# mgp25/OpenLTE

Hardware: AMD Instinct MI355X
Metric: DL subframes/sec @20MHz 100RB 64QAM, full chain FFT->CE->demap->rate-unmatch->turbo(REF)->CRC (SURVEY 8d W4) (higher is better)
Workload: dtype i8 IQ in, f32 FFT/CE/equaliser, i8 soft bits, i16 path metrics (differences exact modulo 2^16); 1 GPU; W4 full DL chain: 20 MHz/100 RB/64QAM, 9 allocations per subframe (8x12 PRB TBS 3240 + 1x4 PRB TBS 1064), 65536 subframes per GPU, int8 IQ in HBM; subframes_per_gpu=65536, N_ant=1, CFI=2, channel_estimate_form=compact, decoder=REF (reference-faithful, bit-exact), unique_subframes=96, streams_per_gpu=1

## Files before the change

### openlte_amd/csrc/turbo.hip

```cpp
#include <algorithm>
#include <cstring>
#include <initializer_list>
#include <type_traits>
#include <vector>

#include "plan_core.hpp"
#include "turbo_swar.h"

using namespace turbo_geom;

namespace {

constexpr uint32_t RX_NULL_AS_INT = 10000;


__device__ __forceinline__ int sbyte(uint32_t w, int k) { return (int)__builtin_amdgcn_sbfe(w, 8 * k, 8); }

typedef __attribute__((address_space(3))) const uint8_t  lds_u8_t;
typedef __attribute__((address_space(3))) const int8_t   lds_i8_t;
typedef __attribute__((address_space(3))) const uint16_t lds_u16_t;
__device__ __forceinline__ uint32_t lds_u8(uint32_t addr) { return *(lds_u8_t *)(uintptr_t)addr; }
__device__ __forceinline__ int      lds_i8(uint32_t addr) { return *(lds_i8_t *)(uintptr_t)addr; }
__device__ __forceinline__ uint32_t lds_u16(uint32_t addr) { return *(lds_u16_t *)(uintptr_t)addr; }

// ... 663 lines not shown
            mtab1[t] = (int8_t)(int)(127.0f * (w / W1));
            mtab2[t] = (int8_t)(int)(127.0f * (w / W2));
        }
        __syncthreads();
    }
    if (nv >= 0) {
        *reinterpret_cast<uint4 *>(out.arr[4] + unit_off(tile_off, lane, u)) = closed(w1max) ? closed16(w1, w1max) : lookup16(0, w1);
        *reinterpret_cast<uint4 *>(out.arr[5] + unit_off(tile_off, lane, u)) = closed(w2max) ? closed16(w2, w2max) : lookup16(MTAB_N, w2);
    }
}


struct SisoPass {
    const uint8_t *in_a;
    const uint8_t *in_b;
    const uint8_t *mag;
    uint8_t       *out;
    uint32_t      *dec;
};
struct SisoArgs { SisoPass p[2]; };

typedef unsigned short v2u __attribute__((ext_vector_type(2)));
__device__ __forceinline__ uint32_t sign_bits(v2s n) { return __builtin_bit_cast(uint32_t, __builtin_bit_cast(v2u, n) >> 15); }

template <int S> __device__ __forceinline__ void acs_step2(v2s (&pm)[8], v2s x2, v2s y2, uint32_t &acc)
{
    const v2s mx = as_v2s(neg_mask(x2 ^ y2)), nmx = ~mx;
    const v2s uP = (x2 + y2) & nmx;
    const v2s uQ = (x2 - y2) & mx;
    const uint32_t m0p = neg_mask(x2) & 0xFFF8FFF8u;
    const v2s P2 = as_v2s(__builtin_amdgcn_bitop3_b32(as_u32(mx), m0p, 0xFFFCFFFCu, 0x06));
    const v2s Q2 = as_v2s(__builtin_amdgcn_bitop3_b32(as_u32(mx), m0p, 0xFFFCFFFCu, 0x60));
// ... 10 lines not shown
    nw[1] = sel(n1 - Q2, pm[3] + uQ, pm[2] - uQ);
    nw[5] = sel(n1 + Q2, pm[3] - uQ, pm[2] + uQ);
    nw[2] = sel(n2 + Q2, pm[5] - uQ, pm[4] + uQ);
    nw[6] = sel(n2 - Q2, pm[5] + uQ, pm[4] - uQ);
    nw[3] = sel(n3 + P2, pm[7] - uP, pm[6] + uP);
    nw[7] = sel(n3 - P2, pm[7] + uP, pm[6] - uP);
#pragma unroll
    for (int s = 0; s < 8; s++) pm[s] = nw[s];
}

template <int R> __device__ __forceinline__ v2s byte_pair2(uint32_t w0, uint32_t w1)
{
    return as_v2s(__builtin_amdgcn_perm(w1, w0, (uint32_t)(4 + R) << 24 | 0x0C0000u | (uint32_t)R << 8 | 0x0Cu)) >> 7;
}

__device__ __forceinline__ uint32_t traceback_entry(uint32_t byte, uint32_t cur)
{
    uint32_t mask = 0;
    for (int k = 0; k < 2; k++) {
        const uint32_t nib = k ? byte >> 4 : byte & 15u;
        const uint32_t j = cur & 3u, bit = (nib >> (3 - j)) & 1u, st = 2 * j + bit;
        const bool     pos = (cur < st) || (cur == st && cur == 0);
        if (!pos) mask |= k ? 0x00FFu : 0xFF00u;
        cur = st;
    }
    return cur | mask << 8;
}

#ifndef SISO_WPE
#define SISO_WPE 4
#endif
template <bool MULTI>
__global__ __launch_bounds__(256) __attribute__((amdgpu_waves_per_eu(SISO_WPE, 8))) void k_turbo_siso(SisoArgs args, uint32_t K_arg, uint32_t n_tiles_arg, uint32_t mode, MultiArgs ma,
                                                                                                         const uint32_t *__restrict__ order)
{
    __shared__ uint32_t tb_lut[2048];
    for (uint32_t i = threadIdx.x; i < 2048; i += blockDim.x) tb_lut[i] = traceback_entry(i >> 3, i & 7u);
    __syncthreads();
    const uint32_t lane = threadIdx.x & 63u;
    uint32_t       K = K_arg, n_tiles = n_tiles_arg, wv = blockIdx.x * 4 + (threadIdx.x >> 6), n_wv = mode ? n_tiles : (n_tiles + 1) / 2;
    size_t         seg_off = 0;
    if constexpr (MULTI) {
        if (order) wv = __builtin_amdgcn_readfirstlane(order[wv]);
        if (wv >= n_tiles_arg) return;
        const_seg_t &sg = multi_seg(ma, wv);
        K = sg.K; n_tiles = sg.n_tiles; seg_off = sg.arr_off;
        wv -= mode ? sg.wv23 : sg.wv1;
        n_wv = mode ? n_tiles : (n_tiles + 1) / 2;
    }
    const uint32_t Kp = kpad64(K), nblk = Kp >> 6;
    if (wv >= n_wv) return;
    const uint8_t *pa[2], *pb[2], *pmag[2];
    uint8_t       *pout[2];
    uint32_t      *dec[2];
#pragma unroll
    for (int h = 0; h < 2; h++) {
        const SisoPass &ps   = args.p[mode ? h : 0];
        const uint32_t  tile = mode ? wv : min(2 * wv + h, n_tiles - 1);
        const size_t    off  = seg_off + (size_t)tile * Kp * 64 + lane * 64;
        pa[h] = ps.in_a + off; pb[h] = ps.in_b + off; pmag[h] = ps.mag + off; pout[h] = ps.out + off;
        dec[h] = ps.dec + (seg_off >> 3) + ((size_t)tile * nblk * 64 + lane) * 8;
    }

    v2s pm[8];
#pragma unroll
    for (int s = 0; s < 8; s++) pm[s] = (v2s)(0);

    uint4 A[2][4], B[2][4];
#pragma unroll
    for (int h = 0; h < 2; h++)
#pragma unroll
        for (int q = 0; q < 4; q++) {
            A[h][q] = reinterpret_cast<const uint4 *>(pa[h])[q];
            B[h][q] = reinterpret_cast<const uint4 *>(pb[h])[q];
        }
    for (uint32_t blk = 0; blk < nblk; blk++) {
        const uint32_t nxt = (blk + 1 < nblk) ? blk + 1 : blk;
        uint32_t       dw[2][8];
#pragma unroll
        for (int q = 0; q < 4; q++) {
#pragma unroll
            for (int g2 = 0; g2 < 2; g2++) {
                const int g = 2 * q + g2;
                uint32_t  acc_lo = 0, acc_hi = 0;
                if (blk * 64 + g * 8 < K) {
                    const uint32_t a0l = g2 ? A[0][q].z : A[0][q].x, a0h = g2 ? A[0][q].w : A[0][q].y;
                    const uint32_t a1l = g2 ? A[1][q].z : A[1][q].x, a1h = g2 ? A[1][q].w : A[1][q].y;
                    const uint32_t b0l = g2 ? B[0][q].z : B[0][q].x, b0h = g2 ? B[0][q].w : B[0][q].y;
                    const uint32_t b1l = g2 ? B[1][q].z : B[1][q].x, b1h = g2 ? B[1][q].w : B[1][q].y;
                    acs_step2<0>(pm, byte_pair2<0>(a0l, a1l), byte_pair2<0>(b0l, b1l), acc_lo);
                    acs_step2<1>(pm, byte_pair2<1>(a0l, a1l), byte_pair2<1>(b0l, b1l), acc_lo);
                    acs_step2<2>(pm, byte_pair2<2>(a0l, a1l), byte_pair2<2>(b0l, b1l), acc_lo);
                    acs_step2<3>(pm, byte_pair2<3>(a0l, a1l), byte_pair2<3>(b0l, b1l), acc_lo);
                    acs_step2<0>(pm, byte_pair2<0>(a0h, a1h), byte_pair2<0>(b0h, b1h), acc_hi);
                    acs_step2<1>(pm, byte_pair2<1>(a0h, a1h), byte_pair2<1>(b0h, b1h), acc_hi);
                    acs_step2<2>(pm, byte_pair2<2>(a0h, a1h), byte_pair2<2>(b0h, b1h), acc_hi);
                    acs_step2<3>(pm, byte_pair2<3>(a0h, a1h), byte_pair2<3>(b0h, b1h), acc_hi);
                }
                dw[0][g] = __builtin_amdgcn_perm(acc_lo, acc_hi, 0x05040100u);
                dw[1][g] = __builtin_amdgcn_perm(acc_lo, acc_hi, 0x07060302u);
            }
            if (q >= 2) {
#pragma unroll
                for (int qq = (q == 2 ? 0 : 3); qq <= (q == 2 ? 2 : 3); qq++)
#pragma unroll
                    for (int h = 0; h < 2; h++) {
                        A[h][qq] = reinterpret_cast<const uint4 *>(pa[h] + (size_t)nxt * 4096)[qq];
                        B[h][qq] = reinterpret_cast<const uint4 *>(pb[h] + (size_t)nxt * 4096)[qq];
                    }
            }
        }
#pragma unroll
        for (int h = 0; h < 2; h++) {
            uint4 *dp = reinterpret_cast<uint4 *>(dec[h] + (size_t)blk * 64 * 8);
            dp[0] = make_uint4(dw[h][0], dw[h][1], dw[h][2], dw[h][3]);
            dp[1] = make_uint4(dw[h][4], dw[h][5], dw[h][6], dw[h][7]);
        }
    }

    int cur[2] = {0, 0};
    {
        int best[2] = {0, 0};
#pragma unroll
        for (int s = 1; s < 8; s++) {
            const uint32_t d  = as_u32(pm[s] - pm[0]);
            const int      dh[2] = {(int)__builtin_amdgcn_sbfe(d, 0, 16), (int)d >> 16};
#pragma unroll
            for (int h = 0; h < 2; h++)
                if (dh[h] < best[h]) { best[h] = dh[h]; cur[h] = s; }
        }
    }

    uint4 M[2][4], Mn[2][4], D[2][2], Dn[2][2];
#pragma unroll
    for (int h = 0; h < 2; h++) {
        const uint4 *dp = reinterpret_cast<const uint4 *>(dec[h] + (size_t)(nblk - 1) * 64 * 8);
        D[h][0] = dp[0];
        D[h][1] = dp[1];
#pragma unroll
        for (int q = 0; q < 4; q++) M[h][q] = reinterpret_cast<const uint4 *>(pmag[h] + (size_t)(nblk - 1) * 4096)[q];
    }
    for (int blk = (int)nblk - 1; blk >= 0; blk--) {
        const int prv = blk > 0 ? blk - 1 : 0;
#pragma unroll
        for (int h = 0; h < 2; h++) {
            const uint4 *dpn = reinterpret_cast<const uint4 *>(dec[h] + (size_t)prv * 64 * 8);
            Dn[h][0] = dpn[0];
            Dn[h][1] = dpn[1];
#pragma unroll
            for (int q = 0; q < 4; q++) Mn[h][q] = reinterpret_cast<const uint4 *>(pmag[h] + (size_t)prv * 4096)[q];
        }
#pragma unroll
        for (int q = 3; q >= 0; q--) {
            uint32_t ow[2][4];
#pragma unroll
            for (int g2 = 1; g2 >= 0; g2--) {
                const int g = 2 * q + g2;
                uint32_t  o_hi[2] = {0, 0}, o_lo[2] = {0, 0};
                if ((uint32_t)blk * 64 + g * 8 < K) {
                    uint32_t word[2], mlo[2], mhi[2], msk[2][4];
#pragma unroll
                    for (int h = 0; h < 2; h++) {
                        const uint4 dq = D[h][g >> 2];
                        word[h] = (g & 3) == 0 ? dq.x : (g & 3) == 1 ? dq.y : (g & 3) == 2 ? dq.z : dq.w;
                        mlo[h]  = g2 ? M[h][q].z : M[h][q].x;
                        mhi[h]  = g2 ? M[h][q].w : M[h][q].y;
                    }
#pragma unroll
                    for (int b = 0; b < 4; b++) {
#pragma unroll
                        for (int h = 0; h < 2; h++) {
                            const uint32_t e = tb_lut[((word[h] >> (8 * b)) & 0xFFu) << 3 | (uint32_t)cur[h]];
                            cur[h]    = (int)(e & 7u);
                            msk[h][b] = e >> 8;
                        }
                    }
#pragma unroll
                    for (int h = 0; h < 2; h++) {
                        o_hi[h] = turbo_swar::joined_from(mhi[h], msk[h][0] << 16 | msk[h][1]);
                        o_lo[h] = turbo_swar::joined_from(mlo[h], msk[h][2] << 16 | msk[h][3]);
                    }
                }
#pragma unroll
                for (int h = 0; h < 2; h++) { ow[h][2 * g2] = o_lo[h]; ow[h][2 * g2 + 1] = o_hi[h]; }
            }
#pragma unroll
            for (int h = 0; h < 2; h++)
                reinterpret_cast<uint4 *>(pout[h] + (size_t)blk * 4096)[q] = make_uint4(ow[h][0], ow[h][1], ow[h][2], ow[h][3]);
        }
#pragma unroll
        for (int h = 0; h < 2; h++) {
            D[h][0] = Dn[h][0];
            D[h][1] = Dn[h][1];
#pragma unroll
            for (int q = 0; q < 4; q++) M[h][q] = Mn[h][q];
        }
    }
}

struct SmallPar { uint32_t cw, uw; };

__device__ __forceinline__ uint2 map_compose(uint2 F, uint2 G)
{
    return make_uint2(__builtin_amdgcn_perm(F.y, F.x, G.x), __builtin_amdgcn_perm(F.y, F.x, G.y));
}
__device__ __forceinline__ uint32_t map_at(uint2 F, uint32_t s) { return ((s & 4u ? F.y : F.x) >> (8 * (s & 3u))) & 7u; }
template <int N> __device__ __forceinline__ uint2 map_row_shl(uint2 v, uint2 keep)
{
    return make_uint2((uint32_t)__builtin_amdgcn_update_dpp((int)keep.x, (int)v.x, 0x100 + N, 0xF, 0xF, false),
                      (uint32_t)__builtin_amdgcn_update_dpp((int)keep.y, (int)v.y, 0x100 + N, 0xF, 0xF, false));
// ... 98 lines not shown
    {
        const uint32_t q0 = (uint32_t)__builtin_amdgcn_mov_dpp((int)XY, 0x00, 0xF, 0xF, false), q1 = (uint32_t)__builtin_amdgcn_mov_dpp((int)XY, 0x55, 0xF, 0xF, false);
        const uint32_t q2 = (uint32_t)__builtin_amdgcn_mov_dpp((int)XY, 0xAA, 0xF, 0xF, false), q3 = (uint32_t)__builtin_amdgcn_mov_dpp((int)XY, 0xFF, 0xF, 0xF, false);
        const short pm[8] = {(short)q0, (short)q1, (short)q2, (short)q3, (short)(q0 >> 16), (short)(q1 >> 16), (short)(q2 >> 16), (short)(q3 >> 16)};
        int best = 0;
#pragma unroll
        for (int st = 1; st < 8; st++) {
            const int d = (short)(pm[st] - pm[0]);
            if (d < best) { best = d; cur = st; }
        }
    }

    const uint2 MAP_ID = make_uint2(0x03020100u, 0x07060504u);
    for (uint32_t g = 0; g < n_g; g++) {
        uint32_t       end = (uint32_t)__builtin_amdgcn_readlane((int)cur, (int)(g * 4));
        const uint8_t *mag = pass_of(g).mag + off_of(g);
        uint8_t       *out = pass_of(g).out + off_of(g);
        uint8_t m_nxt = mag[(size_t)(n_chunk - 1) * 4096 + lane];
        for (int ch = (int)n_chunk - 1; ch >= 0; ch--) {
            const uint32_t t = (uint32_t)ch * 64 + lane;
            const uint8_t  m = m_nxt;
            if (ch > 0) m_nxt = mag[(size_t)(ch - 1) * 4096 + lane];
            const uint4    w = *reinterpret_cast<const uint4 *>(&decw[(g * n_w32 + (t >> 5)) * 4]);
            const uint32_t sh = 31u - (t & 31u);
            uint2          G = MAP_ID;
            if (t < K) {
                const uint32_t f = 0x06040200u + (((w.x >> sh) & 1u) | ((w.y >> sh) & 1u) << 8 | ((w.z >> sh) & 1u) << 16 | ((w.w >> sh) & 1u) << 24);
                G = make_uint2(f, f);
            }
            G = map_compose(G, map_row_shl<1>(G, MAP_ID));
            G = map_compose(G, map_row_shl<2>(G, MAP_ID));
            G = map_compose(G, map_row_shl<4>(G, MAP_ID));
            G = map_compose(G, map_row_shl<8>(G, MAP_ID));
            const uint32_t row = lane >> 4;
#pragma unroll
            for (int r = 1; r < 4; r++) {
                const uint2 R = make_uint2((uint32_t)__builtin_amdgcn_readlane((int)G.x, 16 * r), (uint32_t)__builtin_amdgcn_readlane((int)G.y, 16 * r));
                if (row < (uint32_t)r) G = map_compose(G, R);
            }
            const uint2    Gn  = make_uint2((uint32_t)__shfl_down((int)G.x, 1u), (uint32_t)__shfl_down((int)G.y, 1u));
            const uint32_t nxt = lane == 63 ? end : map_at(Gn, end);
            const uint32_t st  = map_at(G, end);
            if (t < K) {
                const bool    pos = (nxt < st) || (nxt == st && nxt == 0);
                out[(size_t)ch * 4096 + lane] = (pos || m == 0) ? m : (uint8_t)(m | 0x80u);
            }
            end = (uint32_t)__builtin_amdgcn_readlane((int)st, 0);
        }
    }
}

namespace sw = turbo_swar;
struct UnitWords { uint32_t w[5]; };
__device__ __forceinline__ UnitWords load_unit_words(const uint8_t *arr, size_t tile_off, uint32_t lane, uint32_t u)
{
    const uint4 c    = *reinterpret_cast<const uint4 *>(arr + unit_off(tile_off, lane, u));
    uint32_t    prev = 0x7F7F7F7Fu;
    if (u > 0) prev = *reinterpret_cast<const uint32_t *>(arr + unit_off(tile_off, lane, u - 1) + 12);
    return UnitWords{{prev, c.x, c.y, c.z, c.w}};
}
struct PermArgs { const uint8_t *A1; const uint8_t *X2; uint8_t *out[2];  };

#ifndef PERM_NB
#define PERM_NB 4
#endif
static_assert(PERM_NB == PERM_BLOCKS, "a size's perm grid is a multiple of 128 workgroups (the merged decode's map granularity) only for four blocks per workgroup");
template <int NSLOT, bool MULTI = false>
__global__ __launch_bounds__(384) void k_turbo_perm(PermArgs a, uint32_t K_arg, uint32_t n_cb_arg, const uint16_t *__restrict__ pi_arg, MultiArgs ma)
{
    static_assert(NSLOT == 1, "one unit per thread");
    uint32_t K = K_arg, n_cb = n_cb_arg, bidx = blockIdx.x, grid = gridDim.x;
    size_t   seg_off = 0;
    const uint16_t *__restrict__ pi = pi_arg;
    if constexpr (MULTI) {
        const_seg_t &sg = multi_seg(ma, blockIdx.x >> 7);
        K = sg.K; n_cb = sg.n_cb; pi = (const uint16_t *)sg.pi; bidx = blockIdx.x - sg.wg_perm; grid = sg.perm_grid;
// ... 15 lines not shown
#pragma unroll 1
    for (uint32_t it = 0; it < PERM_NB; it++) {
        const uint32_t cb = xcd_cb(bidx + it * grid, n_cb), tile = cb >> 6, lane = cb & 63;
        const size_t   tile_off = seg_off + (size_t)tile * Kp * 64;
        if (cb >= n_cb) {
            if (MULTI && cb < ((n_cb + 63u) & ~63u) && nv >= 0) {
                *reinterpret_cast<uint4 *>(a.out[0] + unit_off(tile_off, lane, u0)) = make_uint4(0, 0, 0, 0);
                *reinterpret_cast<uint4 *>(a.out[1] + unit_off(tile_off, lane, u0)) = make_uint4(0, 0, 0, 0);
            }
            continue;
        }
        uint32_t u = u0;
        asm volatile("" : "+v"(u), "+v"(praw.lo.x), "+v"(praw.lo.y), "+v"(praw.lo.z), "+v"(praw.lo.w), "+v"(praw.hi.x), "+v"(praw.hi.y), "+v"(praw.hi.z), "+v"(praw.hi.w));
        uint4          X2 = make_uint4(0, 0, 0, 0);
        if (nv >= 0) {
            const UnitWords wa = load_unit_words(a.A1, tile_off, lane, u);
            uint32_t        pa = wa.w[0];
            X2 = *reinterpret_cast<const uint4 *>(a.X2 + unit_off(tile_off, lane, u));
            uint32_t c1[4];
#pragma unroll
            for (int j = 0; j < 4; j++) {
                const uint32_t ja = wa.w[j + 1];
                const sw::SM4  A  = sw::unjoin(ja);
                c1[j] = (4 * j < nv) ? sw::to_tc(sw::step3(A, sw::feedback(ja, pa))) : 0u;
                pa    = ja;
            }
            *reinterpret_cast<uint4 *>(sm + 16 * u) = make_uint4(c1[0], c1[1], c1[2], c1[3]);
        }
        __syncthreads();
        uint4 I1 = make_uint4(0, 0, 0, 0);
        if (nv > 0) {
// ... 12 lines not shown
            for (int j = 0; j < 4; j++) {
                const uint32_t p = pack4u(w[4 * j], w[4 * j + 1], w[4 * j + 2], w[4 * j + 3]);
                o[j] = wmax == 254 ? (p >> 1) & 0x7F7F7F7Fu : p;
            }
            if (nv >= 0) *reinterpret_cast<uint4 *>(a.out[1] + unit_off(tile_off, lane, u)) = make_uint4(o[0], o[1], o[2], o[3]);
            continue;
        }
        const float W = (float)wmax;
        for (uint32_t t = threadIdx.x; t < MTAB_N; t += blockDim.x) mtab[t] = (int8_t)(int)(127.0f * ((float)t / W));
        __syncthreads();
        if (nv >= 0) *reinterpret_cast<uint4 *>(a.out[1] + unit_off(tile_off, lane, u)) = lookup16(0, w);
        __syncthreads();
    }
}

struct VoteArgs { const uint8_t *X0, *A1, *B1, *B2; };

template <bool GROUP, int NSLOT, bool MULTI = false>
__global__ __launch_bounds__(384) __attribute__((amdgpu_waves_per_eu(6, 8))) void k_turbo_vote(VoteArgs a, uint32_t K_arg, uint32_t n_cb_arg, const uint16_t *__restrict__ inv_arg,
                                                    uint8_t *__restrict__ c_bits, GroupDesc g, MultiArgs ma)
{
    static_assert(NSLOT == 1, "one unit per thread");
    uint32_t K = K_arg, n_cb = n_cb_arg, bidx = blockIdx.x;
    size_t   seg_off = 0;
    const uint16_t *__restrict__ inv = inv_arg;
    if constexpr (MULTI) {
        const_seg_t &sg = multi_seg(ma, blockIdx.x >> 9);
        K = sg.K; n_cb = sg.n_cb; inv = (const uint16_t *)sg.inv2; bidx = blockIdx.x - sg.wg_cb; seg_off = sg.arr_off;
        g.desc += sg.cb_base;
    }
    extern __shared__ __attribute__((aligned(16))) int8_t sm[];
// ... 2 lines not shown
    const size_t   tile_off = seg_off + (size_t)tile * Kp * 64;
    int8_t        *d12 = sm, *bits = sm + 2 * Kp + 32;
    uint32_t      *red_u = reinterpret_cast<uint32_t *>(bits + Kp);
    const uint32_t u  = threadIdx.x;
    const int      nv = (u < n_units) ? min(16, max(0, (int)K - 16 * (int)u)) : -1;
    IdxRaw vraw;
    {
        const uint4 *ip = reinterpret_cast<const uint4 *>(inv + 16 * (size_t)(nv > 0 ? u : 0));
        vraw.lo = ip[0];
        vraw.hi = ip[1];
    }
    const uint32_t crc_w0 = (GROUP && nv > 0) ? g.crc_tab[MI_CRC_TAB_BIAS + K - 16 * u - 16] : 0u;
    v2s            s0e[4], s0o[4];
    if (threadIdx.x == 0) *reinterpret_cast<uint32_t *>(d12 + 2 * Kp) = 0u;
    if (nv >= 0) {
        const UnitWords wa = load_unit_words(a.A1, tile_off, lane, u), wb = load_unit_words(a.B1, tile_off, lane, u),
                        wc = load_unit_words(a.B2, tile_off, lane, u);
        uint32_t        pa = wa.w[0], pb = wb.w[0], pc = wc.w[0];
        const uint4    x0 = *reinterpret_cast<const uint4 *>(a.X0 + unit_off(tile_off, lane, u));
        const uint32_t x0w[4] = {x0.x, x0.y, x0.z, x0.w};
        uint32_t       dn[8];
#pragma unroll
        for (int j = 0; j < 4; j++) {
            const uint32_t ja = wa.w[j + 1], jb = wb.w[j + 1], jc = wc.w[j + 1];
            const sw::SM4  A = sw::unjoin(ja), B = sw::unjoin(jb), B_ = sw::unjoin(jc);
            const sw::SM4  F  = sw::feedback(ja, pa);
            const sw::SM4  G  = sw::feedback(jb, pb);
            const sw::SM4  G_ = sw::feedback(jc, pc);
            pa = ja; pb = jb; pc = jc;
            const uint32_t u1 = sw::step10_biased(A, B, G), n2 = sw::step11_neg_biased(B_, G_);
            const uint32_t de = sw::sub_halves(sw::even_halves(u1), sw::even_halves(n2)), dd = sw::sub_halves(sw::odd_halves(u1), sw::odd_halves(n2));
            const uint32_t x0b = x0w[j] ^ sw::HI, nc = sw::step3_neg_biased(A, F);
// ... 328 lines not shown
                uint32_t v = 0;
                for (uint32_t b = 0; b < 8; b++) v = v << 1 | ((8 * m + b < tbs) ? (c[F + 8 * m + b] & 1u) : 0u);
                o[m] = (uint8_t)v;
            }
    }
    crc = wave_xor_u(crc);
    if ((threadIdx.x & 63) == 0) red[threadIdx.x >> 6] = crc;
    __syncthreads();
    if (threadIdx.x == 0) g.status[alloc] = ((red[0] ^ red[1] ^ red[2] ^ red[3]) == 0) ? 0 : 2;
}

}


namespace {
enum { AX0, AX1, AX2, AI0, AM1, AM2, AA1, AI1, AM3, AB1, AB2 };
static_assert(sizeof(CbDesc) == CB_DESC_BYTES, "ref_scratch_bytes counts a descriptor per slot");
}

extern "C" size_t mi_lte_turbo_scratch_bytes(uint32_t K, uint32_t n_cb)
{
    const size_t n_tiles = (n_cb + 63) / 64;
    return ref_scratch_bytes(n_tiles * kpad64(K) * 64, n_tiles * 64);
}

static bool no_static_lds(std::initializer_list<const void *> kernels)
{
    hipFuncAttributes a;
    for (const void *k : kernels)
        if (hipFuncGetAttributes(&a, k) != hipSuccess || a.sharedSizeBytes != 0) return false;
    return true;
}

struct RefScratch {
    uint8_t *base;
    CbDesc  *d_desc;
    PrepOut  po;
    SisoArgs s1, s23;
    PermArgs pa;
    VoteArgs va;
    RefScratch(void *scratch, size_t arr_bytes) : base((uint8_t *)scratch)
    {
        uint8_t *arr[N_BYTE_ARRAYS];
        for (int a = 0; a < N_BYTE_ARRAYS; a++) arr[a] = base + a * arr_bytes;
        uint32_t *dec[3];
        for (int p = 0; p < 3; p++) dec[p] = (uint32_t *)(base + N_BYTE_ARRAYS * arr_bytes + p * (arr_bytes / 2));
        d_desc = (CbDesc *)(base + N_BYTE_ARRAYS * arr_bytes + 3 * (arr_bytes / 2));
        po.arr[0] = arr[AX0]; po.arr[1] = arr[AX1]; po.arr[2] = arr[AX2];
        po.arr[3] = arr[AI0]; po.arr[4] = arr[AM1]; po.arr[5] = arr[AM2];
        s1.p[0] = {arr[AX1], arr[AX0], arr[AM1], arr[AA1], dec[0]};
        s1.p[1] = s1.p[0];
        pa.A1 = arr[AA1]; pa.X2 = arr[AX2]; pa.out[0] = arr[AI1]; pa.out[1] = arr[AM3];
        s23.p[0] = {arr[AX2], arr[AI0], arr[AM2], arr[AB1], dec[1]};
        s23.p[1] = {arr[AX2], arr[AI1], arr[AM3], arr[AB2], dec[2]};
        va = {arr[AX0], arr[AA1], arr[AB1], arr[AB2]};
    }
};

template <typename Src, bool GROUP>
static int turbo_ref_run(mi_lte_ctx *ctx, Src src, uint32_t K, uint32_t n_cb, uint8_t *d_c_bits, GroupDesc gd, uint32_t e_cap = 0)
{
    TurboTables tb;
    int         rc = mi_ctx_turbo_tables(ctx, K, 0, &tb);
    if (rc != MI_LTE_OK) return rc;
    static const bool lds_ok = no_static_lds({(const void *)k_turbo_prep<Src, 1>, (const void *)k_turbo_perm<1>, (const void *)k_turbo_vote<GROUP, 1>});
    if (!lds_ok) { ctx->err = "turbo kernels were built with static LDS: absolute LDS addressing is invalid"; return MI_LTE_ERR_HIP; }
    const size_t n_tiles = (n_cb + 63) / 64, Kp = kpad64(K), arr_bytes = n_tiles * Kp * 64;
    rc = mi_ctx_reserve_scratch(ctx, ref_scratch_bytes(arr_bytes, n_tiles * 64));
    if (rc != MI_LTE_OK) return rc;
    const RefScratch sc(ctx->scratch, arr_bytes);
// ... 1 lines not shown
    if (n_cb % 64 && !small)
        MI_HIP_CHECK(ctx, hipMemsetAsync(sc.base, 0, N_BYTE_ARRAYS * arr_bytes, ctx->stream));

    if constexpr (GROUP) {
        gd.desc = src.g.desc = sc.d_desc;
        MI_LAUNCH(ctx, "k_cb_desc", k_cb_desc, dim3((n_cb + 255) / 256), dim3(256), 0, gd, n_cb, (const uint32_t *)src.nnn, sc.d_desc);
    }
    const uint32_t cb_threads = cb_width(K);
    MI_LAUNCH(ctx, "k_turbo_prep", (k_turbo_prep<Src, 1>), dim3(cb_grid(n_cb)), dim3(cb_threads), prep_lds_bytes(Kp, e_cap), src, K, n_cb, tb.d_pi, sc.po, MultiArgs{});

    auto lds_of = [&](uint32_t gpw) { return siso_small_lds_bytes(gpw, Kp); };
    if (small)
        MI_LAUNCH(ctx, "k_turbo_siso_small", k_turbo_siso_small<false>, dim3((n_cb + gpw_of(n_cb) - 1) / gpw_of(n_cb)), dim3(64), lds_of(gpw_of(n_cb)), sc.s1, K, n_cb, 0u,
                  gpw_of(n_cb), MultiArgs{});
    else
        MI_LAUNCH(ctx, "k_turbo_siso", k_turbo_siso<false>, dim3(((n_tiles + 1) / 2 + 3) / 4), dim3(256), 0, sc.s1, K, (uint32_t)n_tiles, 0u, MultiArgs{}, (const uint32_t *)nullptr);

    MI_LAUNCH(ctx, "k_turbo_perm", k_turbo_perm<1>, dim3(perm_grid_of(n_cb)), dim3(cb_threads), MTAB_N + Kp + 32, sc.pa, K, n_cb, tb.d_pi, MultiArgs{});

    if (small)
        MI_LAUNCH(ctx, "k_turbo_siso_small", k_turbo_siso_small<false>, dim3((2 * n_cb + gpw_of(2 * n_cb) - 1) / gpw_of(2 * n_cb)), dim3(64), lds_of(gpw_of(2 * n_cb)), sc.s23, K,
                  n_cb, 1u, gpw_of(2 * n_cb), MultiArgs{});
    else
        MI_LAUNCH(ctx, "k_turbo_siso", k_turbo_siso<false>, dim3((n_tiles + 3) / 4), dim3(256), 0, sc.s23, K, (uint32_t)n_tiles, 1u, MultiArgs{}, (const uint32_t *)nullptr);

    MI_LAUNCH(ctx, "k_turbo_vote", (k_turbo_vote<GROUP, 1>), dim3(cb_grid(n_cb)), dim3(cb_threads), 3 * Kp + 64, sc.va, K, n_cb, tb.d_inv2, d_c_bits, gd, MultiArgs{});
    MI_HIP_CHECK(ctx, hipGetLastError());
    ctx->last_kernels = "k_turbo_prep:1,k_turbo_siso:2,k_turbo_perm:1,k_turbo_vote:1";
    return MI_LTE_OK;
}

template <typename T>
static int turbo_ref_batch(mi_lte_ctx *ctx, const T *d_soft, uint32_t K, uint32_t n_cb, uint8_t *d_c_bits)
{
    SrcDirect<T> src{0, d_soft, nullptr};
    GroupDesc    none{};
    return turbo_ref_run<SrcDirect<T>, false>(ctx, src, K, n_cb, d_c_bits, none);
}

// ... 105 lines not shown
                s1.tabs = rt.d_tabs; s1.nnn = rt.d_nnn; s1.g.desc = sc.d_desc + gr.cb_base; s1.e_cap = G.e_cap_one[c];
                PrepOut p1 = sc.po;
                for (int a = 0; a < 6; a++) p1.arr[a] += G.off_one[c];
                MI_LAUNCH(ctx, "k_turbo_prep", (k_turbo_prep<SrcRateUnmatchPk, 1, false>), dim3(G.grid_cb[c]), dim3(64 * (c + 1)), G.lds_prep[c], s1, gr.K, gr.n_cb, (const uint16_t *)tb.d_pi,
                          p1, MultiArgs{});
                continue;
            }
            MI_LAUNCH(ctx, "k_turbo_prep", (k_turbo_prep<SrcRateUnmatchPk, 1, true>), dim3(G.grid_cb[c]), dim3(64 * (c + 1)), G.lds_prep[c], src, 0u, 0u, (const uint16_t *)nullptr, sc.po,
                      (MultiArgs{d_segs, d_map + G.map_cb[c]}));
        }
    const bool small = G.n_slots <= ctx->siso_small_max;
    auto lds_small = [&](uint32_t gpw) { return siso_small_lds_bytes(gpw, G.kp_all); };
    if (small)
        MI_LAUNCH(ctx, "k_turbo_siso_small", k_turbo_siso_small<true>, dim3(G.n_ws1), dim3(64), lds_small(G.gpw1), sc.s1, 0u, 0u, 0u, G.gpw1, (MultiArgs{d_segs, d_map + G.map_ws1}));
    else
    MI_LAUNCH(ctx, "k_turbo_siso", k_turbo_siso<true>, dim3(G.n_ord1 ? G.n_ord1 / 4 : (G.n_wv1 + 3) / 4), dim3(256), G.siso_pad1, sc.s1, 0u, G.n_wv1, 0u, (MultiArgs{d_segs, d_map + G.map_wv1}),
              G.n_ord1 ? d_map + G.ord_wv1 : (const uint32_t *)nullptr);
    for (int c = 0; c < NCLS; c++)
        if (G.grid_perm[c])
            MI_LAUNCH(ctx, "k_turbo_perm", (k_turbo_perm<1, true>), dim3(G.grid_perm[c]), dim3(64 * (c + 1)), MTAB_N + G.kp_max[c] + 32, sc.pa, 0u, 0u, (const uint16_t *)nullptr,
                      (MultiArgs{d_segs, d_map + G.map_perm[c]}));
    if (small)
        MI_LAUNCH(ctx, "k_turbo_siso_small", k_turbo_siso_small<true>, dim3(G.n_ws23), dim3(64), lds_small(G.gpw23), sc.s23, 0u, 0u, 1u, G.gpw23, (MultiArgs{d_segs, d_map + G.map_ws23}));
    else
    MI_LAUNCH(ctx, "k_turbo_siso", k_turbo_siso<true>, dim3(G.n_ord23 ? G.n_ord23 / 4 : (G.n_wv23 + 3) / 4), dim3(256), G.siso_pad23, sc.s23, 0u, G.n_wv23, 1u, (MultiArgs{d_segs, d_map + G.map_wv23}),
              G.n_ord23 ? d_map + G.ord_wv23 : (const uint32_t *)nullptr);
    for (int c = 0; c < NCLS; c++)
        if (G.grid_cb[c])
            MI_LAUNCH(ctx, "k_turbo_vote", (k_turbo_vote<true, 1, true>), dim3(G.grid_cb[c]), dim3(64 * (c + 1)), 3 * G.kp_max[c] + 64, sc.va, 0u, 0u, (const uint16_t *)nullptr,
                      (uint8_t *)nullptr, gd, (MultiArgs{d_segs, d_map + G.map_cb[c]}));
    MI_HIP_CHECK(ctx, hipGetLastError());
    return MI_LTE_OK;
}

int mi_turbo_ref_dispatch(mi_lte_ctx *ctx, const MiKGroup *groups, uint32_t n_groups, const MiDecodeIO &io, MiMultiCache *cache)
{
    std::vector<MiKGroup> take;
    if (ctx->merged_decode)
        for (uint32_t i = 0; i < n_groups; i++)
            if (mi_turbo_ref_multi_takes(groups[i].K, groups[i].e_max)) take.push_back(groups[i]);
// ... 99 lines not shown
```

### openlte_amd/csrc/turbo_plan.hpp

```cpp
#pragma once

#include <cstddef>
#include <cstdint>
#include <vector>

#ifdef __HIPCC__
#define MI_HD __host__ __device__
#else
#define MI_HD
#endif
#ifdef __clang__
#define MI_GLOBAL_AS __attribute__((address_space(1)))
#else
#define MI_GLOBAL_AS
#endif

namespace turbo_geom {

MI_HD inline uint32_t kpad64(uint32_t K) { return (K + 63u) & ~63u; }

MI_HD inline uint32_t xcd_chunk(uint32_t n_cb) { return ((((n_cb + 63u) >> 6) + 7u) >> 3) << 6; }
MI_HD inline uint32_t xcd_cb(uint32_t b, uint32_t n_cb) { return (b & 7u) * xcd_chunk(n_cb) + (b >> 3); }
inline uint32_t cb_grid(uint32_t n_cb) { return 8 * xcd_chunk(n_cb); }

// ... 11 lines not shown
constexpr uint32_t QTAB_N = 4096;
constexpr uint32_t QTAB_HALF = 2048;
constexpr uint32_t MTAB_N = 256;
constexpr uint32_t PREP_RED_AT = 2 * MTAB_N, PREP_E_AT = PREP_RED_AT + 64, PREP_QTAB_AT = PREP_E_AT, PREP_Q0_AT = PREP_QTAB_AT + QTAB_N;
MI_HD constexpr uint32_t prep_lds_bytes(uint32_t Kp, uint32_t e_cap) { return PREP_E_AT + (e_cap > QTAB_N + Kp ? e_cap : QTAB_N + Kp); }
inline uint32_t stage_cap(uint32_t e_max_bytes) { return (e_max_bytes + 16u + 63u) & ~63u; }
inline bool prep_stages(uint32_t K, uint32_t cap) { return prep_lds_bytes(kpad64(K), cap) <= 48 * 1024; }
inline uint32_t merged_e_cap(uint32_t K, uint32_t e_max_bytes)
{
    const uint32_t cap = stage_cap(e_max_bytes), cap_w = (uint32_t)((15 * (size_t)(K + 4) / 4 + 64 + 63) & ~(size_t)63);
    return prep_stages(K, cap) ? (kpad64(K) <= 1024 ? (cap < cap_w ? cap : cap_w) : cap) : cap_w;
}

inline bool mi_turbo_ref_multi_takes(uint32_t K, uint32_t e_max_bytes) { return (e_max_bytes + (3 * K - 81) - 1) / (3 * K - 81) <= 258; }

constexpr int    N_BYTE_ARRAYS = 11;
constexpr size_t CB_DESC_BYTES = 32;
inline size_t ref_scratch_bytes(size_t arr_bytes, size_t n_slots) { return N_BYTE_ARRAYS * arr_bytes + 3 * (arr_bytes / 2) + ((n_slots + 63) & ~(size_t)63) * CB_DESC_BYTES; }

}

struct MiKGroup { uint32_t K, n_cb, cb_base, e_max; };

struct KSeg {
    uint32_t        K, n_cb, cb_base, n_tiles;
    uint32_t        wg_cb;
    uint32_t        wg_perm, perm_grid;
    uint32_t        e_cap;
    uint32_t        wv1, wv23;
    uint64_t        arr_off;
    MI_GLOBAL_AS const uint16_t *pi, *inv2, *tabs;
    MI_GLOBAL_AS const uint32_t *nnn;
    uint32_t        ws1, ws23;
// ... 21 lines not shown
```

### openlte_amd/csrc/turbo_swar.h

```cpp
#pragma once

#include <cstdint>

#ifdef __HIPCC__
#define SWAR_FN __host__ __device__ __forceinline__
#else
#define SWAR_FN inline
#endif

namespace turbo_swar {

constexpr uint32_t HI = 0x80808080u, LO7 = 0x7F7F7F7Fu, ONES = 0x01010101u, EVEN = 0x00FF00FFu;

SWAR_FN uint32_t alignbit(uint32_t hi, uint32_t lo, uint32_t sh)
{
#if defined(__HIP_DEVICE_COMPILE__)
    return __builtin_amdgcn_alignbit(hi, lo, sh);
#else
    return (uint32_t)((((uint64_t)hi << 32) | lo) >> sh);
#endif
}
SWAR_FN uint32_t sub_halves(uint32_t a, uint32_t b)
{
#if defined(__HIP_DEVICE_COMPILE__)
// ... 2 lines not shown
#else
    return ((a - (b & 0xFFFFu)) & 0xFFFFu) | ((a & 0xFFFF0000u) - (b & 0xFFFF0000u));
#endif
}

struct SM4 { uint32_t m, s; };

SWAR_FN uint32_t low7(uint32_t bits) { return bits - (bits >> 7); }

SWAR_FN uint32_t to_joined(uint32_t w)
{
    const uint32_t s = w & HI, t = s >> 7;
    return (w ^ (s - t)) + t;
}
SWAR_FN uint32_t joined_from(uint32_t m, uint32_t neg_mask) { return m | (neg_mask & (m + LO7) & HI); }
SWAR_FN SM4 unjoin(uint32_t j) { return SM4{j & LO7, j & HI}; }
SWAR_FN SM4 split(uint32_t w) { return unjoin(to_joined(w)); }
SWAR_FN uint32_t join(const SM4 &a) { return a.m | a.s; }
SWAR_FN uint32_t to_tc(const SM4 &a)
{
    const uint32_t t = a.s >> 7;
    return ((a.m ^ (a.s - t)) + t) | a.s;
}

SWAR_FN uint32_t biased(uint32_t x, uint32_t neg)
{
    const uint32_t t = neg >> 7;
    return ((x ^ (neg - t)) + t) + (neg ^ HI);
}
SWAR_FN uint32_t even_halves(uint32_t w) { return w & EVEN; }
// ... 23 lines not shown

SWAR_FN uint32_t step10_biased(const SM4 &A, const SM4 &B, const SM4 &G)
{
    const uint32_t mx = B.s ^ G.s, tm = mx >> 7, m7 = mx - tm;
    const uint32_t y  = (A.m & m7) | (B.m & ~m7);
    const uint32_t w  = avg_biased(G.m | HI, biased(y, mx & (A.s ^ B.s)));
    return (w ^ (m7 | mx)) + tm;
}
SWAR_FN uint32_t step11_neg_biased(const SM4 &B, const SM4 &G)
{
    const uint32_t mx = B.s ^ G.s, tm = mx >> 7, m7 = mx - tm;
    const uint32_t w  = avg_biased(B.m | HI, biased(G.m, mx & B.s));
    return (w ^ ~(m7 | mx)) + (tm ^ ONES);
}

}
```

Before: 2.764 million subframes/s.

## Store SISO traceback signs as packed bit arrays instead of joined byte outputs

The SISO traceback no longer reads the magnitude array and writes a full byte-per-bit joined output. It writes only packed 1-bit sign masks, built by funnel-shifting LUT bits or by a wave ballot in the small-K path, and the perm and vote kernels rebuild the joined bytes on load from magnitude plus sign bits. Three byte scratch arrays are dropped, which cuts HBM traffic in the traceback. The kernel is also templated on mode, so mode 1 loads only one A input. In exchange, consumers do extra unpacking ALU work and read from two arrays.

```diff
diff --git a/openlte_amd/csrc/turbo.hip b/openlte_amd/csrc/turbo.hip
--- a/openlte_amd/csrc/turbo.hip
+++ b/openlte_amd/csrc/turbo.hip
@@ -701,8 +701,7 @@
 struct SisoPass {
     const uint8_t *in_a;
     const uint8_t *in_b;
-    const uint8_t *mag;
-    uint8_t       *out;
+    uint32_t      *sgn;
     uint32_t      *dec;
 };
 struct SisoArgs { SisoPass p[2]; };
@@ -743,28 +742,18 @@
     return as_v2s(__builtin_amdgcn_perm(w1, w0, (uint32_t)(4 + R) << 24 | 0x0C0000u | (uint32_t)R << 8 | 0x0Cu)) >> 7;
 }
 
-__device__ __forceinline__ uint32_t traceback_entry(uint32_t byte, uint32_t cur)
-{
-    uint32_t mask = 0;
-    for (int k = 0; k < 2; k++) {
-        const uint32_t nib = k ? byte >> 4 : byte & 15u;
-        const uint32_t j = cur & 3u, bit = (nib >> (3 - j)) & 1u, st = 2 * j + bit;
-        const bool     pos = (cur < st) || (cur == st && cur == 0);
-        if (!pos) mask |= k ? 0x00FFu : 0xFF00u;
-        cur = st;
-    }
-    return cur | mask << 8;
-}
 
 #ifndef SISO_WPE
 #define SISO_WPE 4
 #endif
-template <bool MULTI>
-__global__ __launch_bounds__(256) __attribute__((amdgpu_waves_per_eu(SISO_WPE, 8))) void k_turbo_siso(SisoArgs args, uint32_t K_arg, uint32_t n_tiles_arg, uint32_t mode, MultiArgs ma,
+template <bool MULTI, int MODE>
+__global__ __launch_bounds__(256) __attribute__((amdgpu_waves_per_eu(SISO_WPE, 8))) void k_turbo_siso(SisoArgs args, uint32_t K_arg, uint32_t n_tiles_arg, MultiArgs ma,
                                                                                                          const uint32_t *__restrict__ order)
 {
+    constexpr uint32_t mode = MODE;
+    constexpr int      NA = MODE ? 1 : 2;
     __shared__ uint32_t tb_lut[2048];
-    for (uint32_t i = threadIdx.x; i < 2048; i += blockDim.x) tb_lut[i] = traceback_entry(i >> 3, i & 7u);
+    for (uint32_t i = threadIdx.x; i < 2048; i += blockDim.x) tb_lut[i] = turbo_swar::traceback_entry(i >> 3, i & 7u);
     __syncthreads();
     const uint32_t lane = threadIdx.x & 63u;
     uint32_t       K = K_arg, n_tiles = n_tiles_arg, wv = blockIdx.x * 4 + (threadIdx.x >> 6), n_wv = mode ? n_tiles : (n_tiles + 1) / 2;
@@ -779,28 +768,28 @@
     }
     const uint32_t Kp = kpad64(K), nblk = Kp >> 6;
     if (wv >= n_wv) return;
-    const uint8_t *pa[2], *pb[2], *pmag[2];
-    uint8_t       *pout[2];
-    uint32_t      *dec[2];
+    const uint8_t *pa[2], *pb[2];
+    uint32_t      *dec[2], *sgn[2];
 #pragma unroll
     for (int h = 0; h < 2; h++) {
         const SisoPass &ps   = args.p[mode ? h : 0];
         const uint32_t  tile = mode ? wv : min(2 * wv + h, n_tiles - 1);
         const size_t    off  = seg_off + (size_t)tile * Kp * 64 + lane * 64;
-        pa[h] = ps.in_a + off; pb[h] = ps.in_b + off; pmag[h] = ps.mag + off; pout[h] = ps.out + off;
+        pa[h] = ps.in_a + off; pb[h] = ps.in_b + off;
         dec[h] = ps.dec + (seg_off >> 3) + ((size_t)tile * nblk * 64 + lane) * 8;
+        sgn[h] = ps.sgn + (seg_off >> 5) + ((size_t)tile * nblk * 64 + lane) * 2;
     }
 
     v2s pm[8];
 #pragma unroll
     for (int s = 0; s < 8; s++) pm[s] = (v2s)(0);
 
-    uint4 A[2][4], B[2][4];
+    uint4 A[NA][4], B[2][4];
 #pragma unroll
     for (int h = 0; h < 2; h++)
 #pragma unroll
         for (int q = 0; q < 4; q++) {
-            A[h][q] = reinterpret_cast<const uint4 *>(pa[h])[q];
+            if (h < NA) A[h][q] = reinterpret_cast<const uint4 *>(pa[h])[q];
             B[h][q] = reinterpret_cast<const uint4 *>(pb[h])[q];
         }
     for (uint32_t blk = 0; blk < nblk; blk++) {
@@ -814,7 +803,7 @@
                 uint32_t  acc_lo = 0, acc_hi = 0;
                 if (blk * 64 + g * 8 < K) {
                     const uint32_t a0l = g2 ? A[0][q].z : A[0][q].x, a0h = g2 ? A[0][q].w : A[0][q].y;
-                    const uint32_t a1l = g2 ? A[1][q].z : A[1][q].x, a1h = g2 ? A[1][q].w : A[1][q].y;
+                    const uint32_t a1l = g2 ? A[NA - 1][q].z : A[NA - 1][q].x, a1h = g2 ? A[NA - 1][q].w : A[NA - 1][q].y;
                     const uint32_t b0l = g2 ? B[0][q].z : B[0][q].x, b0h = g2 ? B[0][q].w : B[0][q].y;
                     const uint32_t b1l = g2 ? B[1][q].z : B[1][q].x, b1h = g2 ? B[1][q].w : B[1][q].y;
                     acs_step2<0>(pm, byte_pair2<0>(a0l, a1l), byte_pair2<0>(b0l, b1l), acc_lo);
@@ -834,7 +823,7 @@
                 for (int qq = (q == 2 ? 0 : 3); qq <= (q == 2 ? 2 : 3); qq++)
 #pragma unroll
                     for (int h = 0; h < 2; h++) {
-                        A[h][qq] = reinterpret_cast<const uint4 *>(pa[h] + (size_t)nxt * 4096)[qq];
+                        if (h < NA) A[h][qq] = reinterpret_cast<const uint4 *>(pa[h] + (size_t)nxt * 4096)[qq];
                         B[h][qq] = reinterpret_cast<const uint4 *>(pb[h] + (size_t)nxt * 4096)[qq];
                     }
             }
@@ -860,14 +849,12 @@
         }
     }
 
-    uint4 M[2][4], Mn[2][4], D[2][2], Dn[2][2];
+    uint4 D[2][2], Dn[2][2];
 #pragma unroll
     for (int h = 0; h < 2; h++) {
         const uint4 *dp = reinterpret_cast<const uint4 *>(dec[h] + (size_t)(nblk - 1) * 64 * 8);
         D[h][0] = dp[0];
         D[h][1] = dp[1];
-#pragma unroll
-        for (int q = 0; q < 4; q++) M[h][q] = reinterpret_cast<const uint4 *>(pmag[h] + (size_t)(nblk - 1) * 4096)[q];
     }
     for (int blk = (int)nblk - 1; blk >= 0; blk--) {
         const int prv = blk > 0 ? blk - 1 : 0;
@@ -876,53 +863,34 @@
             const uint4 *dpn = reinterpret_cast<const uint4 *>(dec[h] + (size_t)prv * 64 * 8);
             Dn[h][0] = dpn[0];
             Dn[h][1] = dpn[1];
-#pragma unroll
-            for (int q = 0; q < 4; q++) Mn[h][q] = reinterpret_cast<const uint4 *>(pmag[h] + (size_t)prv * 4096)[q];
-        }
-#pragma unroll
-        for (int q = 3; q >= 0; q--) {
-            uint32_t ow[2][4];
-#pragma unroll
-            for (int g2 = 1; g2 >= 0; g2--) {
-                const int g = 2 * q + g2;
-                uint32_t  o_hi[2] = {0, 0}, o_lo[2] = {0, 0};
-                if ((uint32_t)blk * 64 + g * 8 < K) {
-                    uint32_t word[2], mlo[2], mhi[2], msk[2][4];
+        }
+        uint32_t sbits[2][2];
+#pragma unroll
+        for (int g = 7; g >= 0; g--) {
+            if ((g & 3) == 3) sbits[0][g >> 2] = sbits[1][g >> 2] = 0;
+            if ((uint32_t)blk * 64 + g * 8 < K) {
+                uint32_t word[2];
+#pragma unroll
+                for (int h = 0; h < 2; h++) {
+                    const uint4 dq = D[h][g >> 2];
+                    word[h] = (g & 3) == 0 ? dq.x : (g & 3) == 1 ? dq.y : (g & 3) == 2 ? dq.z : dq.w;
+                }
+#pragma unroll
+                for (int b = 0; b < 4; b++) {
 #pragma unroll
                     for (int h = 0; h < 2; h++) {
-                        const uint4 dq = D[h][g >> 2];
-                        word[h] = (g & 3) == 0 ? dq.x : (g & 3) == 1 ? dq.y : (g & 3) == 2 ? dq.z : dq.w;
-                        mlo[h]  = g2 ? M[h][q].z : M[h][q].x;
-                        mhi[h]  = g2 ? M[h][q].w : M[h][q].y;
-                    }
-#pragma unroll
-                    for (int b = 0; b < 4; b++) {
-#pragma unroll
-                        for (int h = 0; h < 2; h++) {
-                            const uint32_t e = tb_lut[((word[h] >> (8 * b)) & 0xFFu) << 3 | (uint32_t)cur[h]];
-                            cur[h]    = (int)(e & 7u);
-                            msk[h][b] = e >> 8;
-                        }
-                    }
-#pragma unroll
-                    for (int h = 0; h < 2; h++) {
-                        o_hi[h] = turbo_swar::joined_from(mhi[h], msk[h][0] << 16 | msk[h][1]);
-                        o_lo[h] = turbo_swar::joined_from(mlo[h], msk[h][2] << 16 | msk[h][3]);
+                        const uint32_t e = tb_lut[((word[h] >> (8 * b)) & 0xFFu) << 3 | (uint32_t)cur[h]];
+                        cur[h]           = (int)(e & 7u);
+                        sbits[h][g >> 2]   = __builtin_amdgcn_alignbit(sbits[h][g >> 2], e, 30);
                     }
                 }
-#pragma unroll
-                for (int h = 0; h < 2; h++) { ow[h][2 * g2] = o_lo[h]; ow[h][2 * g2 + 1] = o_hi[h]; }
-            }
-#pragma unroll
-            for (int h = 0; h < 2; h++)
-                reinterpret_cast<uint4 *>(pout[h] + (size_t)blk * 4096)[q] = make_uint4(ow[h][0], ow[h][1], ow[h][2], ow[h][3]);
+            }
         }
 #pragma unroll
         for (int h = 0; h < 2; h++) {
+            *reinterpret_cast<uint2 *>(sgn[h] + (size_t)blk * 64 * 2) = make_uint2(sbits[h][0], sbits[h][1]);
             D[h][0] = Dn[h][0];
             D[h][1] = Dn[h][1];
-#pragma unroll
-            for (int q = 0; q < 4; q++) M[h][q] = Mn[h][q];
         }
     }
 }
@@ -1051,13 +1019,10 @@
     const uint2 MAP_ID = make_uint2(0x03020100u, 0x07060504u);
     for (uint32_t g = 0; g < n_g; g++) {
         uint32_t       end = (uint32_t)__builtin_amdgcn_readlane((int)cur, (int)(g * 4));
-        const uint8_t *mag = pass_of(g).mag + off_of(g);
-        uint8_t       *out = pass_of(g).out + off_of(g);
-        uint8_t m_nxt = mag[(size_t)(n_chunk - 1) * 4096 + lane];
+        const uint32_t cb  = mode ? (T0 + g) >> 1 : T0 + g;
+        uint32_t      *sgn = pass_of(g).sgn + (seg_off >> 5) + ((size_t)(cb >> 6) * n_chunk * 64 + (cb & 63u)) * 2;
         for (int ch = (int)n_chunk - 1; ch >= 0; ch--) {
             const uint32_t t = (uint32_t)ch * 64 + lane;
-            const uint8_t  m = m_nxt;
-            if (ch > 0) m_nxt = mag[(size_t)(ch - 1) * 4096 + lane];
             const uint4    w = *reinterpret_cast<const uint4 *>(&decw[(g * n_w32 + (t >> 5)) * 4]);
             const uint32_t sh = 31u - (t & 31u);
             uint2          G = MAP_ID;
@@ -1078,10 +1043,9 @@
             const uint2    Gn  = make_uint2((uint32_t)__shfl_down((int)G.x, 1u), (uint32_t)__shfl_down((int)G.y, 1u));
             const uint32_t nxt = lane == 63 ? end : map_at(Gn, end);
             const uint32_t st  = map_at(G, end);
-            if (t < K) {
-                const bool    pos = (nxt < st) || (nxt == st && nxt == 0);
-                out[(size_t)ch * 4096 + lane] = (pos || m == 0) ? m : (uint8_t)(m | 0x80u);
-            }
+            const bool     pos = (nxt < st) || (nxt == st && nxt == 0);
+            const uint64_t neg = __ballot(t < K && !pos);
+            if (lane == 0) *reinterpret_cast<uint2 *>(sgn + (size_t)ch * 64 * 2) = make_uint2((uint32_t)neg, (uint32_t)(neg >> 32));
             end = (uint32_t)__builtin_amdgcn_readlane((int)st, 0);
         }
     }
@@ -1096,7 +1060,20 @@
     if (u > 0) prev = *reinterpret_cast<const uint32_t *>(arr + unit_off(tile_off, lane, u - 1) + 12);
     return UnitWords{{prev, c.x, c.y, c.z, c.w}};
 }
-struct PermArgs { const uint8_t *A1; const uint8_t *X2; uint8_t *out[2];  };
+__device__ __forceinline__ UnitWords load_unit_joined(const uint8_t *mag, const uint32_t *sgn, size_t tile_off, uint32_t lane, uint32_t u)
+{
+    UnitWords      w = load_unit_words(mag, tile_off, lane, u);
+    const uint32_t *sp = sgn + (tile_off >> 5) + ((size_t)(u >> 2) * 64 + lane) * 2;
+    const uint2    c = *reinterpret_cast<const uint2 *>(sp);
+    uint32_t       ph = 0;
+    if ((u & 3u) == 0 && u > 0) ph = sp[1 - 128];
+    const uint32_t b = sw::unit_sign_bits(c.x, c.y, ph, u);
+    if (u > 0) w.w[0] = sw::joined_from_bits(w.w[0], b & 15u);
+#pragma unroll
+    for (int j = 0; j < 4; j++) w.w[j + 1] = sw::joined_from_bits(w.w[j + 1], (b >> (4 * j + 4)) & 15u);
+    return w;
+}
+struct PermArgs { const uint8_t *M1; const uint32_t *S1;  const uint8_t *X2; uint8_t *out[2];  };
 
 #ifndef PERM_NB
 #define PERM_NB 4
@@ -1142,7 +1119,7 @@
         asm volatile("" : "+v"(u), "+v"(praw.lo.x), "+v"(praw.lo.y), "+v"(praw.lo.z), "+v"(praw.lo.w), "+v"(praw.hi.x), "+v"(praw.hi.y), "+v"(praw.hi.z), "+v"(praw.hi.w));
         uint4          X2 = make_uint4(0, 0, 0, 0);
         if (nv >= 0) {
-            const UnitWords wa = load_unit_words(a.A1, tile_off, lane, u);
+            const UnitWords wa = load_unit_joined(a.M1, a.S1, tile_off, lane, u);
             uint32_t        pa = wa.w[0];
             X2 = *reinterpret_cast<const uint4 *>(a.X2 + unit_off(tile_off, lane, u));
             uint32_t c1[4];
@@ -1185,7 +1162,7 @@
     }
 }
 
-struct VoteArgs { const uint8_t *X0, *A1, *B1, *B2; };
+struct VoteArgs { const uint8_t *X0, *M1, *M2, *M3; const uint32_t *S1, *S2, *S3; };
 
 template <bool GROUP, int NSLOT, bool MULTI = false>
 __global__ __launch_bounds__(384) __attribute__((amdgpu_waves_per_eu(6, 8))) void k_turbo_vote(VoteArgs a, uint32_t K_arg, uint32_t n_cb_arg, const uint16_t *__restrict__ inv_arg,
@@ -1218,8 +1195,8 @@
     v2s            s0e[4], s0o[4];
     if (threadIdx.x == 0) *reinterpret_cast<uint32_t *>(d12 + 2 * Kp) = 0u;
     if (nv >= 0) {
-        const UnitWords wa = load_unit_words(a.A1, tile_off, lane, u), wb = load_unit_words(a.B1, tile_off, lane, u),
-                        wc = load_unit_words(a.B2, tile_off, lane, u);
+        const UnitWords wa = load_unit_joined(a.M1, a.S1, tile_off, lane, u), wb = load_unit_joined(a.M2, a.S2, tile_off, lane, u),
+                        wc = load_unit_joined(a.M3, a.S3, tile_off, lane, u);
         uint32_t        pa = wa.w[0], pb = wb.w[0], pc = wc.w[0];
         const uint4    x0 = *reinterpret_cast<const uint4 *>(a.X0 + unit_off(tile_off, lane, u));
         const uint32_t x0w[4] = {x0.x, x0.y, x0.z, x0.w};
@@ -1578,7 +1555,7 @@
 
 
 namespace {
-enum { AX0, AX1, AX2, AI0, AM1, AM2, AA1, AI1, AM3, AB1, AB2 };
+enum { AX0, AX1, AX2, AI0, AM1, AM2, AI1, AM3 };
 static_assert(sizeof(CbDesc) == CB_DESC_BYTES, "ref_scratch_bytes counts a descriptor per slot");
 }
 
@@ -1609,15 +1586,17 @@
         for (int a = 0; a < N_BYTE_ARRAYS; a++) arr[a] = base + a * arr_bytes;
         uint32_t *dec[3];
         for (int p = 0; p < 3; p++) dec[p] = (uint32_t *)(base + N_BYTE_ARRAYS * arr_bytes + p * (arr_bytes / 2));
-        d_desc = (CbDesc *)(base + N_BYTE_ARRAYS * arr_bytes + 3 * (arr_bytes / 2));
+        uint32_t *sgn[3];
+        for (int p = 0; p < 3; p++) sgn[p] = (uint32_t *)(base + N_BYTE_ARRAYS * arr_bytes + 3 * (arr_bytes / 2) + p * (arr_bytes / 8));
+        d_desc = (CbDesc *)(base + N_BYTE_ARRAYS * arr_bytes + 3 * (arr_bytes / 2) + 3 * (arr_bytes / 8));
         po.arr[0] = arr[AX0]; po.arr[1] = arr[AX1]; po.arr[2] = arr[AX2];
         po.arr[3] = arr[AI0]; po.arr[4] = arr[AM1]; po.arr[5] = arr[AM2];
-        s1.p[0] = {arr[AX1], arr[AX0], arr[AM1], arr[AA1], dec[0]};
+        s1.p[0] = {arr[AX1], arr[AX0], sgn[0], dec[0]};
         s1.p[1] = s1.p[0];
-        pa.A1 = arr[AA1]; pa.X2 = arr[AX2]; pa.out[0] = arr[AI1]; pa.out[1] = arr[AM3];
-        s23.p[0] = {arr[AX2], arr[AI0], arr[AM2], arr[AB1], dec[1]};
-        s23.p[1] = {arr[AX2], arr[AI1], arr[AM3], arr[AB2], dec[2]};
-        va = {arr[AX0], arr[AA1], arr[AB1], arr[AB2]};
+        pa.M1 = arr[AM1]; pa.S1 = sgn[0]; pa.X2 = arr[AX2]; pa.out[0] = arr[AI1]; pa.out[1] = arr[AM3];
+        s23.p[0] = {arr[AX2], arr[AI0], sgn[1], dec[1]};
+        s23.p[1] = {arr[AX2], arr[AI1], sgn[2], dec[2]};
+        va = {arr[AX0], arr[AM1], arr[AM2], arr[AM3], sgn[0], sgn[1], sgn[2]};
     }
 };
 
@@ -1649,7 +1628,7 @@
         MI_LAUNCH(ctx, "k_turbo_siso_small", k_turbo_siso_small<false>, dim3((n_cb + gpw_of(n_cb) - 1) / gpw_of(n_cb)), dim3(64), lds_of(gpw_of(n_cb)), sc.s1, K, n_cb, 0u,
                   gpw_of(n_cb), MultiArgs{});
     else
-        MI_LAUNCH(ctx, "k_turbo_siso", k_turbo_siso<false>, dim3(((n_tiles + 1) / 2 + 3) / 4), dim3(256), 0, sc.s1, K, (uint32_t)n_tiles, 0u, MultiArgs{}, (const uint32_t *)nullptr);
+        MI_LAUNCH(ctx, "k_turbo_siso", (k_turbo_siso<false, 0>), dim3(((n_tiles + 1) / 2 + 3) / 4), dim3(256), 0, sc.s1, K, (uint32_t)n_tiles, MultiArgs{}, (const uint32_t *)nullptr);
 
     MI_LAUNCH(ctx, "k_turbo_perm", k_turbo_perm<1>, dim3(perm_grid_of(n_cb)), dim3(cb_threads), MTAB_N + Kp + 32, sc.pa, K, n_cb, tb.d_pi, MultiArgs{});
 
@@ -1657,7 +1636,7 @@
         MI_LAUNCH(ctx, "k_turbo_siso_small", k_turbo_siso_small<false>, dim3((2 * n_cb + gpw_of(2 * n_cb) - 1) / gpw_of(2 * n_cb)), dim3(64), lds_of(gpw_of(2 * n_cb)), sc.s23, K,
                   n_cb, 1u, gpw_of(2 * n_cb), MultiArgs{});
     else
-        MI_LAUNCH(ctx, "k_turbo_siso", k_turbo_siso<false>, dim3((n_tiles + 3) / 4), dim3(256), 0, sc.s23, K, (uint32_t)n_tiles, 1u, MultiArgs{}, (const uint32_t *)nullptr);
+        MI_LAUNCH(ctx, "k_turbo_siso", (k_turbo_siso<false, 1>), dim3((n_tiles + 3) / 4), dim3(256), 0, sc.s23, K, (uint32_t)n_tiles, MultiArgs{}, (const uint32_t *)nullptr);
 
     MI_LAUNCH(ctx, "k_turbo_vote", (k_turbo_vote<GROUP, 1>), dim3(cb_grid(n_cb)), dim3(cb_threads), 3 * Kp + 64, sc.va, K, n_cb, tb.d_inv2, d_c_bits, gd, MultiArgs{});
     MI_HIP_CHECK(ctx, hipGetLastError());
@@ -1793,7 +1772,7 @@
     if (small)
         MI_LAUNCH(ctx, "k_turbo_siso_small", k_turbo_siso_small<true>, dim3(G.n_ws1), dim3(64), lds_small(G.gpw1), sc.s1, 0u, 0u, 0u, G.gpw1, (MultiArgs{d_segs, d_map + G.map_ws1}));
     else
-    MI_LAUNCH(ctx, "k_turbo_siso", k_turbo_siso<true>, dim3(G.n_ord1 ? G.n_ord1 / 4 : (G.n_wv1 + 3) / 4), dim3(256), G.siso_pad1, sc.s1, 0u, G.n_wv1, 0u, (MultiArgs{d_segs, d_map + G.map_wv1}),
+    MI_LAUNCH(ctx, "k_turbo_siso", (k_turbo_siso<true, 0>), dim3(G.n_ord1 ? G.n_ord1 / 4 : (G.n_wv1 + 3) / 4), dim3(256), G.siso_pad1, sc.s1, 0u, G.n_wv1, (MultiArgs{d_segs, d_map + G.map_wv1}),
               G.n_ord1 ? d_map + G.ord_wv1 : (const uint32_t *)nullptr);
     for (int c = 0; c < NCLS; c++)
         if (G.grid_perm[c])
@@ -1802,7 +1781,7 @@
     if (small)
         MI_LAUNCH(ctx, "k_turbo_siso_small", k_turbo_siso_small<true>, dim3(G.n_ws23), dim3(64), lds_small(G.gpw23), sc.s23, 0u, 0u, 1u, G.gpw23, (MultiArgs{d_segs, d_map + G.map_ws23}));
     else
-    MI_LAUNCH(ctx, "k_turbo_siso", k_turbo_siso<true>, dim3(G.n_ord23 ? G.n_ord23 / 4 : (G.n_wv23 + 3) / 4), dim3(256), G.siso_pad23, sc.s23, 0u, G.n_wv23, 1u, (MultiArgs{d_segs, d_map + G.map_wv23}),
+    MI_LAUNCH(ctx, "k_turbo_siso", (k_turbo_siso<true, 1>), dim3(G.n_ord23 ? G.n_ord23 / 4 : (G.n_wv23 + 3) / 4), dim3(256), G.siso_pad23, sc.s23, 0u, G.n_wv23, (MultiArgs{d_segs, d_map + G.map_wv23}),
               G.n_ord23 ? d_map + G.ord_wv23 : (const uint32_t *)nullptr);
     for (int c = 0; c < NCLS; c++)
         if (G.grid_cb[c])
diff --git a/openlte_amd/csrc/turbo_plan.hpp b/openlte_amd/csrc/turbo_plan.hpp
--- a/openlte_amd/csrc/turbo_plan.hpp
+++ b/openlte_amd/csrc/turbo_plan.hpp
@@ -49,9 +49,9 @@
 
 inline bool mi_turbo_ref_multi_takes(uint32_t K, uint32_t e_max_bytes) { return (e_max_bytes + (3 * K - 81) - 1) / (3 * K - 81) <= 258; }
 
-constexpr int    N_BYTE_ARRAYS = 11;
+constexpr int    N_BYTE_ARRAYS = 8;
 constexpr size_t CB_DESC_BYTES = 32;
-inline size_t ref_scratch_bytes(size_t arr_bytes, size_t n_slots) { return N_BYTE_ARRAYS * arr_bytes + 3 * (arr_bytes / 2) + ((n_slots + 63) & ~(size_t)63) * CB_DESC_BYTES; }
+inline size_t ref_scratch_bytes(size_t arr_bytes, size_t n_slots) { return N_BYTE_ARRAYS * arr_bytes + 3 * (arr_bytes / 2) + 3 * (arr_bytes / 8) + ((n_slots + 63) & ~(size_t)63) * CB_DESC_BYTES; }
 
 }
 
diff --git a/openlte_amd/csrc/turbo_swar.h b/openlte_amd/csrc/turbo_swar.h
--- a/openlte_amd/csrc/turbo_swar.h
+++ b/openlte_amd/csrc/turbo_swar.h
@@ -40,6 +40,13 @@
     return (w ^ (s - t)) + t;
 }
 SWAR_FN uint32_t joined_from(uint32_t m, uint32_t neg_mask) { return m | (neg_mask & (m + LO7) & HI); }
+SWAR_FN uint32_t joined_from_bits(uint32_t m, uint32_t nib) { return m | ((nib * 0x10204080u) & (m + LO7) & HI); }
+SWAR_FN uint32_t unit_sign_bits(uint32_t c_lo, uint32_t c_hi, uint32_t prev_hi, uint32_t u)
+{
+    const uint32_t q = u & 3u;
+    const uint64_t c = ((uint64_t)c_hi << 32) | c_lo;
+    return q ? (uint32_t)(c >> (16u * q - 4u)) & 0xFFFFFu : (c_lo & 0xFFFFu) << 4 | prev_hi >> 28;
+}
 SWAR_FN SM4 unjoin(uint32_t j) { return SM4{j & LO7, j & HI}; }
 SWAR_FN SM4 split(uint32_t w) { return unjoin(to_joined(w)); }
 SWAR_FN uint32_t join(const SM4 &a) { return a.m | a.s; }
@@ -93,4 +100,17 @@
     return (w ^ ~(m7 | mx)) + (tm ^ ONES);
 }
 
+SWAR_FN uint32_t traceback_entry(uint32_t byte, uint32_t cur)
+{
+    uint32_t sgn = 0;
+    for (int k = 0; k < 2; k++) {
+        const uint32_t nib = k ? byte >> 4 : byte & 15u;
+        const uint32_t j = cur & 3u, bit = (nib >> (3 - j)) & 1u, st = 2 * j + bit;
+        const bool     pos = (cur < st) || (cur == st && cur == 0);
+        if (!pos) sgn |= k ? 1u << 30 : 1u << 31;
+        cur = st;
+    }
+    return cur | sgn;
 }
+
+}
```

New measurement: 2.848 million subframes/s, median of 6. 3.0% higher.
